# Danderson123/Amira

Hardware: AMD Instinct MI355X
Metric: gene-mers/s to corrected GeneMerGraph (higher is better)
Workload: dtype int32; 1 GPU; synthetic 1M reads x 60 genes, k=5, 20k-gene vocab: build + error-correction sweep (build, filter(3,1), correct, build, clip(5), correct, build); reads_per_gpu=1000000, genes_per_read=60, k=5, vocab=20000, gene_mers_per_gpu=56000000, final_nodes=472478, final_edges=1054844, multi_gpu=n/a

## Files before the change

### amira_amd/csrc/amg_filter.hip

```cpp
#include "amg_rows.h"

__global__ __launch_bounds__(256) void k_filter_nodes(const unsigned int* __restrict__ cov, unsigned char* __restrict__ alive,
                                                      long long n, unsigned int min_cov) {
  const long long q = (long long)blockIdx.x * blockDim.x + threadIdx.x;
  const long long i0 = 4 * q;
  if (i0 >= n) return;
  if (i0 + 4 > n) {
    for (long long i = i0; i < n; ++i)
      if (alive[i] && cov[i] < min_cov) alive[i] = 0;
    return;
  }
  const unsigned int a = reinterpret_cast<const unsigned int*>(alive)[q];
  if (a == 0u) return;
  const uint4 c = reinterpret_cast<const uint4*>(cov)[q];
  unsigned int keep = 0u;
  if (c.x >= min_cov) keep |= 0x000000ffu;
  if (c.y >= min_cov) keep |= 0x0000ff00u;
  if (c.z >= min_cov) keep |= 0x00ff0000u;
  if (c.w >= min_cov) keep |= 0xff000000u;
  if ((a & keep) != a) reinterpret_cast<unsigned int*>(alive)[q] = a & keep;
}

__device__ __forceinline__ void filter_edge(const int* __restrict__ src, const int* __restrict__ tgt,
                                            const unsigned int* __restrict__ cov,
                                            const unsigned char* __restrict__ node_alive,
                                            unsigned char* __restrict__ alive, long long e, unsigned int min_cov) {
  if (!alive[e]) return;
  if ((min_cov > 1 && cov[e] < min_cov) || !node_alive[src[e]] || !node_alive[tgt[e]]) alive[e] = 0;
}

__global__ __launch_bounds__(256) void k_filter_edges(const int* __restrict__ src, const int* __restrict__ tgt,
                                                      const unsigned int* __restrict__ cov,
                                                      const unsigned char* __restrict__ node_alive,
                                                      unsigned char* __restrict__ alive, long long n, unsigned int min_cov) {
  const long long q = (long long)blockIdx.x * blockDim.x + threadIdx.x;
  const long long e0 = 4 * q;
  if (e0 >= n) return;
  if (e0 + 4 > n) {
    for (long long e = e0; e < n; ++e) filter_edge(src, tgt, cov, node_alive, alive, e, min_cov);
    return;
  }
  const unsigned int a = reinterpret_cast<const unsigned int*>(alive)[q];
  if (a == 0u) return;
  const int4 s = reinterpret_cast<const int4*>(src)[q];
  const int4 t = reinterpret_cast<const int4*>(tgt)[q];
  uint4 c = make_uint4(min_cov, min_cov, min_cov, min_cov);
  if (min_cov > 1) c = reinterpret_cast<const uint4*>(cov)[q];
  const bool l0 = a & 0x000000ffu, l1 = a & 0x0000ff00u, l2 = a & 0x00ff0000u, l3 = a & 0xff000000u;
  const unsigned int ns0 = node_alive[l0 ? s.x : 0], ns1 = node_alive[l1 ? s.y : 0], ns2 = node_alive[l2 ? s.z : 0],
                     ns3 = node_alive[l3 ? s.w : 0];
  const unsigned int nt0 = node_alive[l0 ? t.x : 0], nt1 = node_alive[l1 ? t.y : 0], nt2 = node_alive[l2 ? t.z : 0],
                     nt3 = node_alive[l3 ? t.w : 0];
  unsigned int keep = 0u;
  if (ns0 && nt0 && c.x >= min_cov) keep |= 0x000000ffu;
  if (ns1 && nt1 && c.y >= min_cov) keep |= 0x0000ff00u;
  if (ns2 && nt2 && c.z >= min_cov) keep |= 0x00ff0000u;
  if (ns3 && nt3 && c.w >= min_cov) keep |= 0xff000000u;
  if ((a & keep) != a) reinterpret_cast<unsigned int*>(alive)[q] = a & keep;
}

#define READS_PER_WAVE 8
__global__ __launch_bounds__(256) void k_mask_reads(int* __restrict__ tok_node,
                                                    const long long* __restrict__ read_off,
                                                    long long n_reads,
                                                    const unsigned char* __restrict__ node_alive,
                                                    unsigned char* __restrict__ read_fix,
                                                    unsigned long long* __restrict__ win_mask) {
  const long long rbase = ((long long)blockIdx.x * 4 + (threadIdx.x >> 6)) * READS_PER_WAVE;
  if (rbase >= n_reads) return;
  const int lane = threadIdx.x & 63;
  const long long off_l = (lane <= READS_PER_WAVE && rbase + lane <= n_reads) ? read_off[rbase + lane] : 0;
  long long a[READS_PER_WAVE], b[READS_PER_WAVE];
  int v[READS_PER_WAVE];
#pragma unroll
  for (int j = 0; j < READS_PER_WAVE; ++j) {
    a[j] = __shfl(off_l, j, 64);
    b[j] = rbase + j < n_reads ? __shfl(off_l, j + 1, 64) : a[j];
  }
#pragma unroll
  for (int j = 0; j < READS_PER_WAVE; ++j) v[j] = a[j] + lane < b[j] ? tok_node[a[j] + lane] : -1;
  bool dead[READS_PER_WAVE];
#pragma unroll
  for (int j = 0; j < READS_PER_WAVE; ++j) dead[j] = v[j] >= 0 && !node_alive[v[j]];
  unsigned long long mine = 0;
#pragma unroll
  for (int j = 0; j < READS_PER_WAVE; ++j) {
    const unsigned long long m = __ballot(v[j] >= 0 && !dead[j]);
    if (lane == j) mine = m;
  }
  if (lane < READS_PER_WAVE && rbase + lane < n_reads) win_mask[rbase + lane] = mine;
#pragma unroll
  for (int j = 0; j < READS_PER_WAVE; ++j) {
    if (dead[j]) tok_node[a[j] + lane] = -2;
    bool hit = dead[j];
    for (long long t = a[j] + 64 + lane; t < b[j]; t += 64) {
      const int n = tok_node[t];
      if (n >= 0 && !node_alive[n]) {
        tok_node[t] = -2;
        hit = true;
      }
    }
    if (__any(hit) && lane == 0) read_fix[rbase + j] = 1;
  }
}

static int apply_removals(amg_ctx* c, unsigned int min_edge_cov) {
  hipStream_t st = c->stream;
  if (min_edge_cov > 1) live_lists_after_edge_deaths(c);
  else live_lists_after_node_deaths(c);
  if (c->n_edges > 0)
    hipLaunchKernelGGL(k_filter_edges, dim3(nblk(c->n_edges, 4 * 256)), dim3(256), 0, st,
                       c->edge_src.as<int>(), c->edge_tgt.as<int>(), c->edge_cov.as<unsigned int>(),
                       c->node_alive.as<unsigned char>(), c->edge_alive.as<unsigned char>(),
                       c->n_edges, min_edge_cov);
  AMGCHK(c->win_mask.ensure((size_t)(c->n_reads + 2) * sizeof(unsigned long long)));
  if (c->n_reads > 0)
    hipLaunchKernelGGL(k_mask_reads, dim3(nblk(c->n_reads, 4 * READS_PER_WAVE)), dim3(256), 0, st,
                       c->tok_node.as<int>(), c->read_off.as<long long>(), c->n_reads,
                       c->node_alive.as<unsigned char>(), c->read_fix.as<unsigned char>(),
                       c->win_mask.as<unsigned long long>());
  window_masks_made(c);
  return AMG_OK;
}

extern "C" int amg_filter(amg_ctx* c, uint32_t min_node_cov, uint32_t min_edge_cov) {
  NEED_BUILT(c);
  ctx_removal_begins(c);
  stages_reset(c);
  stage_begin(c, "filter");
  if (c->n_nodes > 0)
    hipLaunchKernelGGL(k_filter_nodes, dim3(nblk(c->n_nodes, 4 * 256)), dim3(256), 0, c->stream,
                       c->node_cov.as<unsigned int>(), c->node_alive.as<unsigned char>(),
                       c->n_nodes, min_node_cov);
  AMGCHK(apply_removals(c, min_edge_cov));
  stage_end(c);
  return AMG_OK;
}

__global__ void k_kill_listed(const int* __restrict__ ids, long long n, long long n_nodes,
                              unsigned char* __restrict__ alive) {
  long long i = (long long)blockIdx.x * blockDim.x + threadIdx.x;
  if (i >= n) return;
  int v = ids[i];
  if (v >= 0 && v < n_nodes) alive[v] = 0;
}

extern "C" int amg_remove_nodes(amg_ctx* c, const int32_t* node_ids, int64_t n) {
  NEED_BUILT(c);
  if (n < 0 || (n > 0 && !node_ids)) return amg_fail(AMG_E_ARG, "bad node list");
  if (n == 0) return AMG_OK;
  ctx_removal_begins(c);
  AMGCHK(c->s0.ensure((size_t)n * sizeof(int)));
  HIPCHK(hipMemcpyAsync(c->s0.p, node_ids, (size_t)n * sizeof(int), hipMemcpyHostToDevice, c->stream));
  hipLaunchKernelGGL(k_kill_listed, dim3(nblk(n, 256)), dim3(256), 0, c->stream, c->s0.as<int>(),
                     (long long)n, c->n_nodes, c->node_alive.as<unsigned char>());
  AMGCHK(apply_removals(c, 0));
  HIPCHK(hipStreamSynchronize(c->stream));
  return AMG_OK;
}

extern "C" int amg_remove_edges(amg_ctx* c, const int32_t* edge_ids, int64_t n) {
  NEED_BUILT(c);
  if (n < 0 || (n > 0 && !edge_ids)) return amg_fail(AMG_E_ARG, "bad edge list");
  if (n == 0) return AMG_OK;
  ctx_removal_begins(c);
  AMGCHK(c->s0.ensure((size_t)n * sizeof(int)));
  HIPCHK(hipMemcpyAsync(c->s0.p, edge_ids, (size_t)n * sizeof(int), hipMemcpyHostToDevice, c->stream));
  hipLaunchKernelGGL(k_kill_listed, dim3(nblk(n, 256)), dim3(256), 0, c->stream, c->s0.as<int>(), (long long)n,
                     c->n_edges, c->edge_alive.as<unsigned char>());
  live_lists_after_edge_deaths(c);
  HIPCHK(hipStreamSynchronize(c->stream));
  return AMG_OK;
}

#define CLIP_MAX 64
template <class View>
__global__ void k_clip_mark(View g, long long n_nodes, int min_length, const unsigned long long* __restrict__ acc,
                            const unsigned int* __restrict__ comp_live,
                            const unsigned char* __restrict__ protect,
                            unsigned char* __restrict__ kill) {
  long long i = (long long)blockIdx.x * blockDim.x + threadIdx.x;
  if (i >= n_nodes || !g.n_alive[i]) return;
  int n = (int)i;
  if (node_degree(g, n) != 1) return;
  int d0 = (g.n_first[n] & 1ll) ? -1 : 1;
  int path[CLIP_MAX];
  int len = 0;
  path[len++] = n;
  int tgt = -1, td = 0;
  int r = lin_step(g, n, d0 == -1, &tgt, &td);
  while (r == 2 && tgt != n) {
    if (len >= min_length) return;
    path[len++] = tgt;
    r = lin_step(g, tgt, td == 1, &tgt, &td);
  }
  r = lin_step(g, n, d0 == 1, &tgt, &td);
  while (r == 2 && tgt != n) {
    if (len >= min_length) return;
    path[len++] = tgt;
    r = lin_step(g, tgt, td == 1, &tgt, &td);
  }
  if (!(len > 0 && len < min_length)) return;
  const double thr = ((double)acc[0] / (double)acc[1]) * 1.5;
  bool all_high = true;
  for (int j = 0; j < len; ++j) all_high = all_high && ((double)g.n_cov[path[j]] > thr);
  if (all_high) return;
  if (comp_live) {
    int distinct = 0;
    for (int j = 0; j < len; ++j) {
      bool dup = false;
      for (int q = 0; q < j; ++q) dup = dup || (path[q] == path[j]);
      distinct += dup ? 0 : 1;
    }
    if ((unsigned int)distinct == comp_live[g.n_comp[n]]) return;
  } else {
    bool closed = true;
    for (int j = 0; j < len && closed; ++j)
      for (int side = 0; side < 2 && closed; ++side) {
        const long long row = 2ll * path[j] + side;
        const int cnt = row_count(g, row);
        for (int q = 0; q < cnt && closed; ++q) {
          const int t = row_target(g, row, q);
          bool in = false;
          for (int m = 0; m < len; ++m) in = in || (path[m] == t);
          closed = in;
        }
      }
    if (closed) return;
  }
  for (int j = 0; j < len; ++j)
    if (!protect || !protect[path[j]]) kill[path[j]] = 1;
}

__device__ __forceinline__ void block_add_cov(unsigned long long sum, unsigned long long n, unsigned long long* __restrict__ acc) {
  __shared__ unsigned long long s_part[2][4];
  for (int d = 32; d > 0; d >>= 1) {
    sum += __shfl_xor(sum, d, 64);
    n += __shfl_xor(n, d, 64);
  }
  if ((threadIdx.x & 63) == 0) {
    s_part[0][threadIdx.x >> 6] = sum;
    s_part[1][threadIdx.x >> 6] = n;
  }
  __syncthreads();
  if (threadIdx.x == 0) {
    const unsigned long long n_all = s_part[1][0] + s_part[1][1] + s_part[1][2] + s_part[1][3];
    if (n_all) {
      atomicAdd(&acc[0], s_part[0][0] + s_part[0][1] + s_part[0][2] + s_part[0][3]);
      atomicAdd(&acc[1], n_all);
    }
  }
}

__global__ void k_comp_hist(const int* __restrict__ comp, const unsigned char* __restrict__ alive,
                            const unsigned int* __restrict__ cov, long long n, unsigned int min_cov,
                            unsigned int* __restrict__ live_cnt, unsigned int* __restrict__ high_cnt,
                            unsigned long long* __restrict__ acc ) {
  int cid = -1;
  unsigned int n_live = 0, n_high = 0;
  unsigned long long s_cov = 0, s_n = 0;
  for (long long i = (long long)blockIdx.x * blockDim.x + threadIdx.x; i < n; i += (long long)gridDim.x * blockDim.x) {
    if (!alive[i]) continue;
    if (acc) {
      s_cov += cov[i];
      s_n += 1;
    }
    const int id = comp[i];
    if (id != cid) {
      if (cid >= 0) {
        atomicAdd(&live_cnt[cid], n_live);
        if (high_cnt && n_high) atomicAdd(&high_cnt[cid], n_high);
      }
      cid = id;
      n_live = n_high = 0;
    }
    ++n_live;
    n_high += (high_cnt && cov[i] >= min_cov) ? 1u : 0u;
  }
  const int lane = threadIdx.x & 63;
  if (acc) block_add_cov(s_cov, s_n, acc);
  bool active = cid >= 0;
  unsigned long long todo = __ballot(active);
  while (todo) {
    const int leader = __ffsll((long long)todo) - 1;
    const int lc = __shfl(cid, leader, 64);
    const bool same = active && cid == lc;
    const unsigned long long m = __ballot(same);
    unsigned int sl = same ? n_live : 0u, sh = same ? n_high : 0u;
    for (int d = 32; d > 0; d >>= 1) {
      sl += __shfl_xor(sl, d, 64);
      sh += __shfl_xor(sh, d, 64);
    }
    if (lane == leader) {
      atomicAdd(&live_cnt[lc], sl);
      if (high_cnt && sh) atomicAdd(&high_cnt[lc], sh);
    }
    active = active && !same;
    todo &= ~m;
  }
}

__global__ __launch_bounds__(256) void k_cov_acc(const unsigned char* __restrict__ alive, const unsigned int* __restrict__ cov,
                                                 long long n, unsigned long long* __restrict__ acc) {
  unsigned long long s_cov = 0, s_n = 0;
  for (long long i = (long long)blockIdx.x * blockDim.x + threadIdx.x; i < n; i += (long long)gridDim.x * blockDim.x)
    if (alive[i]) {
      s_cov += cov[i];
      s_n += 1;
    }
  block_add_cov(s_cov, s_n, acc);
}

__global__ void k_scatter_ids(const unsigned char* __restrict__ killed, const long long* __restrict__ pos,
                              long long n, int* __restrict__ out) {
  long long i = (long long)blockIdx.x * blockDim.x + threadIdx.x;
  if (i < n && killed[i]) out[pos[i]] = (int)i;
}

int kill_marks_reserve(amg_ctx* c, ClearList* cl, KillMarks* marks) {
  const long long D = c->n_nodes;
  AMGCHK(c->s0.ensure((size_t)D + 8));
  cl->add(c->s0.p, (size_t)D + 8);
  *marks = KillMarks{c->s0.as<unsigned char>(), D};
  return AMG_OK;
}

int kill_marks_check(const amg_ctx* c, const KillMarks& marks) {
  if (!marks.bytes || marks.bytes != c->s0.p || marks.n != c->n_nodes)
    return amg_fail(AMG_E_STATE, "the kill marks (%lld nodes) are not the ctx's current ones (%lld nodes): something else "
                                 "ran on the ctx between their reservation and their use",
                    marks.n, (long long)c->n_nodes);
  return AMG_OK;
}

int finish_kill(amg_ctx* c, const KillMarks& marks, int64_t* n_removed, int32_t* removed_ids) {
  hipStream_t st = c->stream;
  const long long D = c->n_nodes;
  AMGCHK(kill_marks_check(c, marks));
  AMGCHK(c->s2.ensure((size_t)(D + 2) * sizeof(long long)));
  AMGCHK(prim_exscan_apply_kill(c, marks.bytes, c->node_alive.as<unsigned char>(), c->s2.as<long long>(), (size_t)D));
  long long total = 0;
  {
    FetchList l;
    l.add(c->s2.as<long long>() + D);
    AMGCHK(fetch(c, l, reinterpret_cast<unsigned long long*>(&total)));
  }
  if (n_removed) *n_removed = total;
  if (removed_ids && total > 0) {
    AMGCHK(c->s3.ensure((size_t)total * sizeof(int)));
    hipLaunchKernelGGL(k_scatter_ids, dim3(nblk(D, 256)), dim3(256), 0, st, marks.bytes, c->s2.as<long long>(), D,
                       c->s3.as<int>());
    HIPCHK(hipMemcpyAsync(removed_ids, c->s3.p, (size_t)total * sizeof(int), hipMemcpyDeviceToHost, st));
  }
  if (total > 0) AMGCHK(apply_removals(c, 0));
  if (removed_ids && total > 0) HIPCHK(hipStreamSynchronize(st));
  return AMG_OK;
}

extern "C" int amg_remove_short_linear_paths(amg_ctx* c, int32_t min_length, const uint8_t* protect,
                                             int64_t* n_removed, int32_t* removed_ids) {
  NEED_BUILT(c);
  if (min_length < 1 || min_length > CLIP_MAX)
    return amg_fail(AMG_E_ARG, "min_length must be in [1, %d]", CLIP_MAX);
  hipStream_t st = c->stream;
  const long long D = c->n_nodes;
  if (n_removed) *n_removed = 0;
  if (D == 0) return AMG_OK;
  ctx_removal_begins(c);
  stages_reset(c);
  const bool by_labels = !c->pristine || getenv("AMG_CLIP_COMPONENTS");
  if (by_labels) AMGCHK(ensure_components(c));
  const bool light = c->live_lists == LiveLists::Absent && !getenv("AMG_CLIP_LISTS");
  stage_begin(c, "clip");
  unsigned long long* acc = c->status.as<unsigned long long>() + ST_COV_SUM;
  KillMarks marks;
  {
    ClearList cl;
    cl.add(acc, 2 * sizeof(unsigned long long));
    AMGCHK(kill_marks_reserve(c, &cl, &marks));
    if (by_labels) {
      AMGCHK(c->s4.ensure((size_t)(c->n_components + 2) * sizeof(unsigned int)));
      cl.add(c->s4.p, (size_t)(c->n_components + 2) * sizeof(unsigned int));
    }
    if (light) AMGCHK(row_summary_reserve(c, &cl));
    AMGCHK(clear_many(c, cl));
  }
  RView summary;
  if (light) summary = row_summary(c);
  if (by_labels)
    hipLaunchKernelGGL(k_comp_hist, dim3(nblk(D, 256) < 256u ? nblk(D, 256) : 256u), dim3(256), 0, st, c->node_comp.as<int>(),
                       c->node_alive.as<unsigned char>(), c->node_cov.as<unsigned int>(), D, 0u,
                       c->s4.as<unsigned int>(), (unsigned int*)nullptr, acc);
  else
    hipLaunchKernelGGL(k_cov_acc, dim3(nblk(D, 2048) < 256u ? nblk(D, 2048) : 256u), dim3(256), 0, st,
                       c->node_alive.as<unsigned char>(), c->node_cov.as<unsigned int>(), D, acc);
  unsigned char* d_protect = nullptr;
  if (protect) {
    AMGCHK(c->s5.ensure((size_t)D + 8));
    HIPCHK(hipMemcpyAsync(c->s5.p, protect, (size_t)D, hipMemcpyHostToDevice, st));
    d_protect = c->s5.as<unsigned char>();
  }
  const unsigned int* comp_live = by_labels ? c->s4.as<unsigned int>() : nullptr;
  if (light) {
    hipLaunchKernelGGL(k_clip_mark<RView>, dim3(nblk(D, 128)), dim3(128), 0, st, summary, D, (int)min_length, acc, comp_live,
                       d_protect, marks.bytes);
  } else {
    AMGCHK(ensure_live_adj(c));
    hipLaunchKernelGGL(k_clip_mark<GView>, dim3(nblk(D, 128)), dim3(128), 0, st, make_view(c), D, (int)min_length, acc,
                       comp_live, d_protect, marks.bytes);
  }
  int r = finish_kill(c, marks, n_removed, removed_ids);
  stage_end(c);
  return r;
}

__global__ void k_kill_low_components(const int* __restrict__ comp, const unsigned char* __restrict__ alive,
                                      const unsigned int* __restrict__ high_cnt, long long n,
                                      unsigned char* __restrict__ kill) {
  long long i = (long long)blockIdx.x * blockDim.x + threadIdx.x;
  if (i < n && alive[i] && high_cnt[comp[i]] == 0) kill[i] = 1;
}

extern "C" int amg_remove_low_coverage_components(amg_ctx* c, uint32_t min_cov) {
  NEED_BUILT(c);
  hipStream_t st = c->stream;
  const long long D = c->n_nodes;
  if (D == 0) return AMG_OK;
  ctx_removal_begins(c);
  AMGCHK(ensure_components(c));
  size_t nc = (size_t)(c->n_components + 2);
  KillMarks marks;
  {
    ClearList cl;
    AMGCHK(kill_marks_reserve(c, &cl, &marks));
    AMGCHK(c->s4.ensure(2 * nc * sizeof(unsigned int)));
    cl.add(c->s4.p, 2 * nc * sizeof(unsigned int));
    AMGCHK(clear_many(c, cl));
  }
  unsigned int* live = c->s4.as<unsigned int>();
  unsigned int* high = live + nc;
  hipLaunchKernelGGL(k_comp_hist, dim3(nblk(D, 256) < 256u ? nblk(D, 256) : 256u), dim3(256), 0, st, c->node_comp.as<int>(),
                     c->node_alive.as<unsigned char>(), c->node_cov.as<unsigned int>(), D, min_cov, live, high,
                     (unsigned long long*)nullptr);
  hipLaunchKernelGGL(k_kill_low_components, dim3(nblk(D, 256)), dim3(256), 0, st, c->node_comp.as<int>(),
                     c->node_alive.as<unsigned char>(), high, D, marks.bytes);
  return finish_kill(c, marks, nullptr, nullptr);
}
```

Before: 10.94 billion gene-mers/s.

## Scan read tokens in contiguous wave chunks and derive per-read masks from ballots

k_mask_reads no longer walks each read separately. Each wave now takes 16 reads and sweeps their concatenated token range in chunks of 64x16 tokens with fully coalesced loads. It ballots live and dead bits per row into shared memory, and each lane then extracts its own read's window mask and dead-hit flag with bit operations. This removes divergent per-read loops and lanes left idle on short reads, in exchange for extra shared-memory traffic, wave barriers and more complex boundary handling.

New measurement: 11.07 billion gene-mers/s (median of 6 runs). +1.1%, better.

```diff
diff --git a/amira_amd/csrc/amg_filter.hip b/amira_amd/csrc/amg_filter.hip
--- a/amira_amd/csrc/amg_filter.hip
+++ b/amira_amd/csrc/amg_filter.hip
@@ -59,48 +59,99 @@
   if ((a & keep) != a) reinterpret_cast<unsigned int*>(alive)[q] = a & keep;
 }
 
-#define READS_PER_WAVE 8
+#define READS_PER_WAVE 16
+#define MASK_ROWS 16
+
+__device__ __forceinline__ unsigned long long mask_bits_from(const unsigned int* w, int s) {
+  const int i = s >> 5, sh = s & 31;
+  const unsigned long long lo = (unsigned long long)w[i] | ((unsigned long long)w[i + 1] << 32);
+  return sh ? (lo >> sh) | ((unsigned long long)w[i + 2] << (64 - sh)) : lo;
+}
+
+__device__ __forceinline__ long long mask_wave_same(long long v) {
+  const unsigned int lo = (unsigned int)__builtin_amdgcn_readfirstlane((int)(unsigned int)(unsigned long long)v);
+  const unsigned int hi = (unsigned int)__builtin_amdgcn_readfirstlane((int)(unsigned int)((unsigned long long)v >> 32));
+  return (long long)(((unsigned long long)hi << 32) | lo);
+}
+
 __global__ __launch_bounds__(256) void k_mask_reads(int* __restrict__ tok_node,
                                                     const long long* __restrict__ read_off,
                                                     long long n_reads,
                                                     const unsigned char* __restrict__ node_alive,
                                                     unsigned char* __restrict__ read_fix,
                                                     unsigned long long* __restrict__ win_mask) {
-  const long long rbase = ((long long)blockIdx.x * 4 + (threadIdx.x >> 6)) * READS_PER_WAVE;
-  if (rbase >= n_reads) return;
-  const int lane = threadIdx.x & 63;
-  const long long off_l = (lane <= READS_PER_WAVE && rbase + lane <= n_reads) ? read_off[rbase + lane] : 0;
-  long long a[READS_PER_WAVE], b[READS_PER_WAVE];
-  int v[READS_PER_WAVE];
+  constexpr int R = READS_PER_WAVE, ROWS = MASK_ROWS, CH = 64 * ROWS;
+  __shared__ unsigned long long s_live[4][ROWS + 1], s_dead[4][ROWS + 1];
+  const int wv = threadIdx.x >> 6, lane = threadIdx.x & 63;
+  const long long r0 = ((long long)blockIdx.x * 4 + wv) * R;
+  if (r0 >= n_reads) return;
+  const int nr = n_reads - r0 < R ? (int)(n_reads - r0) : R;
+  long long lo = 0, hi = 0;
+  if (lane < nr) {
+    lo = read_off[r0 + lane];
+    hi = read_off[r0 + lane + 1];
+  }
+  const long long t0 = mask_wave_same(__shfl(lo, 0, 64)), t1 = mask_wave_same(__shfl(hi, nr - 1, 64));
+  unsigned long long mine = 0;
+  bool hit = false;
+  for (long long base = t0 & ~3ll; base < t1; base += CH) {
+    const int own_lo = t0 > base ? (int)(t0 - base) : 0, own_hi = t1 - base < CH ? (int)(t1 - base) : CH;
+    int v[ROWS];
 #pragma unroll
-  for (int j = 0; j < READS_PER_WAVE; ++j) {
-    a[j] = __shfl(off_l, j, 64);
-    b[j] = rbase + j < n_reads ? __shfl(off_l, j + 1, 64) : a[j];
-  }
+    for (int i = 0; i < ROWS; ++i) v[i] = i * 64 + lane < own_hi ? tok_node[base + i * 64 + lane] : -1;
+    bool ask[ROWS];
+    unsigned char a[ROWS];
 #pragma unroll
-  for (int j = 0; j < READS_PER_WAVE; ++j) v[j] = a[j] + lane < b[j] ? tok_node[a[j] + lane] : -1;
-  bool dead[READS_PER_WAVE];
+    for (int i = 0; i < ROWS; ++i) {
+      const int p = i * 64 + lane;
+      ask[i] = p >= own_lo && p < own_hi && v[i] >= 0;
+      a[i] = ask[i] ? node_alive[(unsigned int)v[i]] : (unsigned char)1;
+    }
+    unsigned long long row_live = 0, row_dead = 0;
 #pragma unroll
-  for (int j = 0; j < READS_PER_WAVE; ++j) dead[j] = v[j] >= 0 && !node_alive[v[j]];
-  unsigned long long mine = 0;
-#pragma unroll
-  for (int j = 0; j < READS_PER_WAVE; ++j) {
-    const unsigned long long m = __ballot(v[j] >= 0 && !dead[j]);
-    if (lane == j) mine = m;
-  }
-  if (lane < READS_PER_WAVE && rbase + lane < n_reads) win_mask[rbase + lane] = mine;
-#pragma unroll
-  for (int j = 0; j < READS_PER_WAVE; ++j) {
-    if (dead[j]) tok_node[a[j] + lane] = -2;
-    bool hit = dead[j];
-    for (long long t = a[j] + 64 + lane; t < b[j]; t += 64) {
-      const int n = tok_node[t];
-      if (n >= 0 && !node_alive[n]) {
-        tok_node[t] = -2;
-        hit = true;
+    for (int i = 0; i < ROWS; ++i) {
+      const bool d = ask[i] && !a[i];
+      const unsigned long long bl = __ballot(ask[i] && a[i]), bd = __ballot(d);
+      if (lane == i) {
+        row_live = bl;
+        row_dead = bd;
       }
-    }
-    if (__any(hit) && lane == 0) read_fix[rbase + j] = 1;
+      if (d) tok_node[base + i * 64 + lane] = -2;
+    }
+    if (lane <= ROWS) {
+      s_live[wv][lane] = row_live;
+      s_dead[wv][lane] = row_dead;
+    }
+    __builtin_amdgcn_fence(__ATOMIC_ACQ_REL, "wavefront");
+    __builtin_amdgcn_wave_barrier();
+    if (lane < nr) {
+      const unsigned int* live = reinterpret_cast<const unsigned int*>(s_live[wv]);
+      const unsigned int* dead = reinterpret_cast<const unsigned int*>(s_dead[wv]);
+      const int s = lo > base ? (lo - base < CH ? (int)(lo - base) : CH) : 0;
+      const int e = hi > base ? (hi - base < CH ? (int)(hi - base) : CH) : 0;
+      if (s < e) {
+        const int ws = s >> 5, we = (e - 1) >> 5;
+        for (int w = ws; w <= we; ++w) {
+          unsigned int m = dead[w];
+          if (w == ws) m &= ~0u << (s & 31);
+          if (w == we) m &= ~0u >> (31 - ((e - 1) & 31));
+          hit = hit || m != 0u;
+        }
+      }
+      const long long at = base + s - lo;
+      if (s < e && at < 64) {
+        const int n = e - s < 64 - (int)at ? e - s : 64 - (int)at;
+        unsigned long long b = mask_bits_from(live, s);
+        if (n < 64) b &= (1ull << n) - 1ull;
+        mine |= b << (int)at;
+      }
+    }
+    __builtin_amdgcn_fence(__ATOMIC_ACQ_REL, "wavefront");
+    __builtin_amdgcn_wave_barrier();
+  }
+  if (lane < nr) {
+    win_mask[r0 + lane] = mine;
+    if (hit) read_fix[r0 + lane] = 1;
   }
 }
 
```
